# returaj/gan_mpc

Measured on AMD Instinct MI355X. Metric: trajectories/sec (rollout+backward+critic step) at batch=1024, H=50, higher is better.
Workload: dtype f32

## Files before the change

### gan_mpc_amd/csrc/gmpc_linearize_sparse.hip

```cpp
#include <cstdio>
#include <type_traits>

#include "gmpc_launch.h"

typedef float f32x4 __attribute__((ext_vector_type(4)));
typedef unsigned v4u __attribute__((ext_vector_type(4)));
typedef unsigned v2u __attribute__((ext_vector_type(2)));

#define GMPC_LIN_PADROWS 24
#define GMPC_SP_H 200
#define GMPC_SP_Z 200
#define GMPC_SP_STR 220
#define GMPC_SP_CAP 216
#define GMPC_SP_WAVE_BYTES (16 * GMPC_SP_STR * 4 + 3 * GMPC_SP_CAP * 4)
#define GMPC_SP_RD 3
#define GMPC_SP_ROW 256

static bool sparse_form(int L, const int* dims, int n, int m) {
  const int Lh = L - 1;
  if (Lh < 2 || n + m > 32 || n < 1) return false;
  for (int l = 1; l <= Lh; ++l)
    if (dims[l] != GMPC_SP_H) return false;
  return true;
}

__global__ void k_pack_sparse(const float* W, float* dst) {
  const int e = blockIdx.x * blockDim.x + threadIdx.x;
  if (e >= GMPC_SP_H * GMPC_SP_H) return;
  const int i = e / GMPC_SP_H, o = e - i * GMPC_SP_H;
  const int t = i >> 4;
  const int slot = i < 192 ? 64 * (t >> 2) + 4 * (i & 15) + (t & 3) : i;
  dst[(size_t)o * GMPC_SP_ROW + slot] = W[e];
}

size_t gmpc_linsparse_floats(int L, const int* dims, int n, int m) {
  if (!sparse_form(L, dims, n, m)) return 0;
  return (size_t)(L - 2) * (GMPC_SP_H + GMPC_LIN_PADROWS) * GMPC_SP_ROW + GMPC_SP_ROW;
}

void gmpc_linsparse_prepare(const MlpDesc& dyn, int n, int m, float* p, LinPad* out, hipStream_t s) {
  for (int l = 0; l < GMPC_MAX_LAYERS; ++l) out->WSP[l] = nullptr;
  if (!sparse_form(dyn.L, dyn.dims, n, m)) return;
  p = reinterpret_cast<float*>((reinterpret_cast<uintptr_t>(p) + 1023) & ~(uintptr_t)1023);
  for (int l = 1; l < dyn.L - 1; ++l) {
    out->WSP[l] = p;
    hipLaunchKernelGGL(k_pack_sparse, dim3((GMPC_SP_H * GMPC_SP_H + 255) / 256), dim3(256), 0, s, dyn.W[l], p);
    p += (size_t)(GMPC_SP_H + GMPC_LIN_PADROWS) * GMPC_SP_ROW;
  }
}

__global__ __launch_bounds__(GMPC_THREADS, 2) void k_linearize_sparse(
    int NSamp, int T, int n, int m, int Lh, LinPad lp, const uint32_t* masks, const int* active, float* AB,
    int samp_mul, int samp_add) {
  extern __shared__ __attribute__((aligned(16))) char smem[];
  const int lane = threadIdx.x & 63, wave = __builtin_amdgcn_readfirstlane(threadIdx.x >> 6);
  const int g = lane >> 4, l16 = lane & 15;
  const int nm = n + m;
  const int nrow = n < 16 ? n : 16;
  char* wbase = smem + wave * GMPC_SP_WAVE_BYTES;
  float* st = reinterpret_cast<float*>(wbase);
  unsigned* lk = reinterpret_cast<unsigned*>(wbase + 16 * GMPC_SP_STR * 4);
  unsigned* lt = lk + GMPC_SP_CAP;
  if (lane < 16 * 8) st[(lane >> 3) * GMPC_SP_STR + GMPC_SP_H + (lane & 7)] = 0.f;
  if (lane + 64 < 16 * 8) st[((lane + 64) >> 3) * GMPC_SP_STR + GMPC_SP_H + (lane & 7)] = 0.f;

  const int lw = l16 * 16, lwt = (192 + (l16 & 7)) * 4;
  const int ls = l16 * GMPC_SP_STR * 4;
  const int tsel = l16 >= 8 ? 1 : 0;
  const unsigned* lkl = lk + g;
  const unsigned* ltl_ = lt + 2 * g + tsel;
  const int lsn = l16 < n ? l16 * 4 : (1 << 28);
  const __amdgpu_buffer_rsrc_t rsl = __builtin_amdgcn_make_buffer_rsrc(
      const_cast<float*>(lp.WLP), 0, (GMPC_SP_H + GMPC_LIN_PADROWS) * n * (int)sizeof(float), 0x00020000);
  const __amdgpu_buffer_rsrc_t rs0 = __builtin_amdgcn_make_buffer_rsrc(
      const_cast<float*>(lp.WTP[0]), 0, (GMPC_SP_H + GMPC_LIN_PADROWS) * 32 * (int)sizeof(float), 0x00020000);

  constexpr int WPB = GMPC_THREADS / 64;
  for (int s = blockIdx.x * WPB + wave; s < NSamp; s += gridDim.x * WPB) {
    const size_t sid = (size_t)s * samp_mul + samp_add;
    if (active != nullptr && active[sid / T] == 0) continue;
    const uint32_t* mrow = masks + sid * Lh * GMPC_MW;

    auto build = [&](int ml) -> int {
      __builtin_amdgcn_wave_barrier();
      int base = 0;
#pragma unroll
      for (int c = 0; c < 4; ++c) {
        const uint32_t lo = __builtin_amdgcn_readfirstlane(mrow[ml * GMPC_MW + 2 * c]);
        uint32_t hi = c < 3 ? __builtin_amdgcn_readfirstlane(mrow[ml * GMPC_MW + 2 * c + 1]) : 0u;
        const uint32_t lo_m = c < 3 ? lo : (lo & 0xFFu);
        const uint32_t word = lane < 32 ? lo_m : hi;
        const int pos = base + (int)__builtin_amdgcn_mbcnt_hi(hi, __builtin_amdgcn_mbcnt_lo(lo_m, 0u));
        const unsigned u = 64 * c + lane;
        if ((word >> (lane & 31)) & 1u) {
          const bool odd = (u & 1u) != 0;
          lk[pos] = u;
          *reinterpret_cast<v2u*>(lt + 2 * pos) = v2u{odd ? GMPC_SP_Z : u, odd ? u : GMPC_SP_Z};
        }
        base += __builtin_popcount(lo_m) + __builtin_popcount(hi);
      }
      if (lane < 16) {
        lk[base + lane] = GMPC_SP_Z;
        *reinterpret_cast<v2u*>(lt + 2 * (base + lane)) = v2u{GMPC_SP_Z, GMPC_SP_Z};
      }
      __builtin_amdgcn_wave_barrier();
      return base;
    };

    auto layer = [&](int l, auto seedc) __attribute__((always_inline)) {
      constexpr bool seed = decltype(seedc)::value;
      const int np = (build(l) + 3) >> 2;
      const __amdgpu_buffer_rsrc_t wrs = __builtin_amdgcn_make_buffer_rsrc(
          const_cast<float*>(lp.WSP[l]), 0, (GMPC_SP_H + GMPC_LIN_PADROWS) * GMPC_SP_ROW * 4, 0x00020000);
      f32x4 acc[13];
      struct Ops { float w[13]; float b; unsigned k, kt; };
      Ops r[GMPC_SP_RD];
      auto tables = [&](Ops& o, int p) {
        o.k = lkl[4 * p];
        o.kt = ltl_[8 * p];
      };
      auto loads = [&](Ops& o) {
        const int k = (int)o.k, kt = (int)o.kt;
        const int vo = (k << 10) + lw, vt = (kt << 10) + lwt;
#pragma unroll
        for (int q = 0; q < 3; ++q) {
          const v4u a = __builtin_amdgcn_raw_buffer_load_b128(wrs, vo + 256 * q, 0, 0);
          o.w[4 * q] = __uint_as_float(a.x); o.w[4 * q + 1] = __uint_as_float(a.y);
          o.w[4 * q + 2] = __uint_as_float(a.z); o.w[4 * q + 3] = __uint_as_float(a.w);
        }
        o.w[12] = __uint_as_float(__builtin_amdgcn_raw_buffer_load_b32(wrs, vt, 0, 0));
        if constexpr (seed) o.b = __uint_as_float(__builtin_amdgcn_raw_buffer_load_b32(rsl, k * n * 4 + lsn, 0, 0));
        else o.b = st[(ls >> 2) + k];
      };
      auto step = [&](int p, Ops& cur, Ops& ahead2) __attribute__((always_inline)) {
        loads(ahead2);
        tables(cur, p + 3);
        __builtin_amdgcn_sched_barrier(0);
#pragma unroll
        for (int t = 0; t < 13; ++t) acc[t] = __builtin_amdgcn_mfma_f32_16x16x4f32(cur.w[t], cur.b, acc[t], 0, 0, 0);
        __builtin_amdgcn_sched_barrier(0);
      };
      if (np == 0) {
#pragma unroll
        for (int t = 0; t < 13; ++t) acc[t] = f32x4{0.f, 0.f, 0.f, 0.f};
      } else {
        tables(r[0], 0); tables(r[1], 1); tables(r[2], 2);
        loads(r[0]); loads(r[1]);
        loads(r[2]);
        tables(r[0], 3);
        __builtin_amdgcn_sched_barrier(0);
#pragma unroll
        for (int t = 0; t < 13; ++t)
          acc[t] = __builtin_amdgcn_mfma_f32_16x16x4f32(r[0].w[t], r[0].b, f32x4{0.f, 0.f, 0.f, 0.f}, 0, 0, 0);
        __builtin_amdgcn_sched_barrier(0);
        int p = 1;
        for (; p + 3 <= np; p += 3) {
          step(p, r[1], r[0]);
          step(p + 1, r[2], r[1]);
          step(p + 2, r[0], r[2]);
        }
        if (p < np) step(p, r[1], r[0]);
        if (p + 1 < np) step(p + 1, r[2], r[1]);
      }
      mfma_fence<false>(acc[0], acc[1], acc[2], acc[3], acc[4], acc[5], acc[6], acc[7], acc[8], acc[9], acc[10],
                        acc[11], acc[12]);
      __builtin_amdgcn_wave_barrier();
      float* srow = st + l16 * GMPC_SP_STR;
#pragma unroll
      for (int t = 0; t < 12; ++t)
        *reinterpret_cast<f32x4*>(srow + 32 * (t >> 1) + 16 * (t & 1) + 4 * g) = acc[t];
      *reinterpret_cast<f32x4*>(srow + (g < 2 ? 192 : 200) + 4 * g) = acc[12];
      __builtin_amdgcn_wave_barrier();
      if (g < 2) {
        const f32x4 x = *reinterpret_cast<const f32x4*>(srow + 192 + 4 * g);
        const f32x4 y = *reinterpret_cast<const f32x4*>(srow + 208 + 4 * g);
        *reinterpret_cast<f32x4*>(srow + 192 + 4 * g) = x + y;
      }
      __builtin_amdgcn_wave_barrier();
    };
    layer(Lh - 1, std::true_type{});
    for (int l = Lh - 2; l >= 1; --l) layer(l, std::false_type{});

    {
      const int np = (build(0) + 3) >> 2;
      f32x4 acc0 = {0.f, 0.f, 0.f, 0.f}, acc1 = {0.f, 0.f, 0.f, 0.f};
      const bool two = nm > 16;
      struct Ops0 { float w0, w1, b; unsigned k; };
      Ops0 r[GMPC_SP_RD];
      auto tables = [&](Ops0& o, int p) { o.k = lkl[4 * p]; };
      auto loads = [&](Ops0& o) {
        const int vo = (int)(o.k << 7) + l16 * 4;
        o.w0 = __uint_as_float(__builtin_amdgcn_raw_buffer_load_b32(rs0, vo, 0, 0));
        o.w1 = __uint_as_float(__builtin_amdgcn_raw_buffer_load_b32(rs0, vo + 64, 0, 0));
        o.b = st[(ls >> 2) + o.k];
      };
      auto step = [&](int p, Ops0& cur, Ops0& ahead2) __attribute__((always_inline)) {
        loads(ahead2);
        tables(cur, p + 3);
        __builtin_amdgcn_sched_barrier(0);
        acc0 = __builtin_amdgcn_mfma_f32_16x16x4f32(cur.w0, cur.b, acc0, 0, 0, 0);
        acc1 = __builtin_amdgcn_mfma_f32_16x16x4f32(cur.w1, cur.b, acc1, 0, 0, 0);
        __builtin_amdgcn_sched_barrier(0);
      };
      tables(r[0], 0); tables(r[1], 1); tables(r[2], 2);
      loads(r[0]); loads(r[1]);
      int p = 0;
      for (; p + 3 <= np; p += 3) {
        step(p, r[0], r[2]);
        step(p + 1, r[1], r[0]);
        step(p + 2, r[2], r[1]);
      }
      if (p < np) step(p, r[0], r[2]);
      if (p + 1 < np) step(p + 1, r[1], r[0]);
      mfma_fence<false>(acc0, acc1);
      if (l16 < nrow) {
        float* dst = AB + ((size_t)s * n + l16) * nm;
#pragma unroll
        for (int j = 0; j < 4; ++j) {
          const int c = 4 * g + j;
          if (c < nm) dst[c] = acc0[j] + (c == l16 ? 1.0f : 0.0f);
          if (two && c + 16 < nm) dst[c + 16] = acc1[j] + (c + 16 == l16 ? 1.0f : 0.0f);
        }
      }
    }
    __builtin_amdgcn_wave_barrier();
  }
}

int gmpc_launch_linearize_sparse(int NSamp, int T, int n, int m, const MlpDesc& dyn, const LinPad& lp,
                                 const uint32_t* masks, const int* active, float* AB, int samp_mul, int samp_add,
                                 hipStream_t s) {
  const int Lh = dyn.L - 1;
  if (!sparse_form(dyn.L, dyn.dims, n, m) || lp.NT != 7 || lp.NTF != 1 || lp.NGF != 1) return -1;
  if (NSamp <= 0) return 0;
  if (n > 16 && gmpc_launch_linearize_regs_rows(NSamp, T, n, m, dyn, lp, masks, active, AB, samp_mul, samp_add, 16,
                                                s) != 0)
    return -1;
  const size_t lds = (size_t)(GMPC_THREADS / 64) * GMPC_SP_WAVE_BYTES;
  int grid = (NSamp + 3) / 4;
  if (grid > 256 * 2) grid = 256 * 2;
  hipLaunchKernelGGL(k_linearize_sparse, dim3(grid), dim3(GMPC_THREADS), lds, s, NSamp, T, n, m, Lh, lp, masks,
                     active, AB, samp_mul, samp_add);
  return 0;
}
```

Measured before the change: 799,800.

## Software-pipeline sparse linearize across layers and samples with double-buffered index tables

Restructures the sparse linearization kernel so the next layer's (or next sample's) mask index table is built into a second LDS buffer and its first weight loads are issued while the current layer's last MFMAs run. Mask words are now loaded once per lane with a vector load and broadcast via readlane instead of scalar readfirstlane loads, and the next trajectory's active flag is prefetched. This targets the pipeline drain and refill bubble at every layer boundary and sample boundary. It doubles the per-wave index-table LDS footprint and adds considerable control complexity.

```diff
diff --git a/gan_mpc_amd/csrc/gmpc_linearize_sparse.hip b/gan_mpc_amd/csrc/gmpc_linearize_sparse.hip
--- a/gan_mpc_amd/csrc/gmpc_linearize_sparse.hip
+++ b/gan_mpc_amd/csrc/gmpc_linearize_sparse.hip
@@ -12,7 +12,7 @@
 #define GMPC_SP_Z 200
 #define GMPC_SP_STR 220
 #define GMPC_SP_CAP 216
-#define GMPC_SP_WAVE_BYTES (16 * GMPC_SP_STR * 4 + 3 * GMPC_SP_CAP * 4)
+#define GMPC_SP_WAVE_BYTES (16 * GMPC_SP_STR * 4 + 2 * 3 * GMPC_SP_CAP * 4)
 #define GMPC_SP_RD 3
 #define GMPC_SP_ROW 256
 
@@ -48,6 +48,10 @@
     p += (size_t)(GMPC_SP_H + GMPC_LIN_PADROWS) * GMPC_SP_ROW;
   }
 }
+
+struct SpOps { float w[13]; float b; unsigned k, kt; };
+enum { GMPC_SP_SEED = 0, GMPC_SP_HID = 1, GMPC_SP_INP = 2 };
+template <int V> using SpKind = std::integral_constant<int, V>;
 
 __global__ __launch_bounds__(GMPC_THREADS, 2) void k_linearize_sparse(
     int NSamp, int T, int n, int m, int Lh, LinPad lp, const uint32_t* masks, const int* active, float* AB,
@@ -59,109 +63,181 @@
   const int nrow = n < 16 ? n : 16;
   char* wbase = smem + wave * GMPC_SP_WAVE_BYTES;
   float* st = reinterpret_cast<float*>(wbase);
-  unsigned* lk = reinterpret_cast<unsigned*>(wbase + 16 * GMPC_SP_STR * 4);
-  unsigned* lt = lk + GMPC_SP_CAP;
+  unsigned* bc = reinterpret_cast<unsigned*>(wbase + 16 * GMPC_SP_STR * 4);
+  unsigned* bn = bc + 3 * GMPC_SP_CAP;
   if (lane < 16 * 8) st[(lane >> 3) * GMPC_SP_STR + GMPC_SP_H + (lane & 7)] = 0.f;
   if (lane + 64 < 16 * 8) st[((lane + 64) >> 3) * GMPC_SP_STR + GMPC_SP_H + (lane & 7)] = 0.f;
+  __builtin_amdgcn_wave_barrier();
 
   const int lw = l16 * 16, lwt = (192 + (l16 & 7)) * 4;
   const int ls = l16 * GMPC_SP_STR * 4;
   const int tsel = l16 >= 8 ? 1 : 0;
-  const unsigned* lkl = lk + g;
-  const unsigned* ltl_ = lt + 2 * g + tsel;
+  const int tofs = GMPC_SP_CAP + g + tsel;
   const int lsn = l16 < n ? l16 * 4 : (1 << 28);
   const __amdgpu_buffer_rsrc_t rsl = __builtin_amdgcn_make_buffer_rsrc(
       const_cast<float*>(lp.WLP), 0, (GMPC_SP_H + GMPC_LIN_PADROWS) * n * (int)sizeof(float), 0x00020000);
   const __amdgpu_buffer_rsrc_t rs0 = __builtin_amdgcn_make_buffer_rsrc(
       const_cast<float*>(lp.WTP[0]), 0, (GMPC_SP_H + GMPC_LIN_PADROWS) * 32 * (int)sizeof(float), 0x00020000);
-
-  constexpr int WPB = GMPC_THREADS / 64;
-  for (int s = blockIdx.x * WPB + wave; s < NSamp; s += gridDim.x * WPB) {
-    const size_t sid = (size_t)s * samp_mul + samp_add;
-    if (active != nullptr && active[sid / T] == 0) continue;
-    const uint32_t* mrow = masks + sid * Lh * GMPC_MW;
-
-    auto build = [&](int ml) -> int {
-      __builtin_amdgcn_wave_barrier();
-      int base = 0;
-#pragma unroll
-      for (int c = 0; c < 4; ++c) {
-        const uint32_t lo = __builtin_amdgcn_readfirstlane(mrow[ml * GMPC_MW + 2 * c]);
-        uint32_t hi = c < 3 ? __builtin_amdgcn_readfirstlane(mrow[ml * GMPC_MW + 2 * c + 1]) : 0u;
-        const uint32_t lo_m = c < 3 ? lo : (lo & 0xFFu);
-        const uint32_t word = lane < 32 ? lo_m : hi;
-        const int pos = base + (int)__builtin_amdgcn_mbcnt_hi(hi, __builtin_amdgcn_mbcnt_lo(lo_m, 0u));
-        const unsigned u = 64 * c + lane;
-        if ((word >> (lane & 31)) & 1u) {
-          const bool odd = (u & 1u) != 0;
-          lk[pos] = u;
-          *reinterpret_cast<v2u*>(lt + 2 * pos) = v2u{odd ? GMPC_SP_Z : u, odd ? u : GMPC_SP_Z};
+  auto wres = [&](int l) {
+    return __builtin_amdgcn_make_buffer_rsrc(const_cast<float*>(lp.WSP[l]), 0,
+                                             (GMPC_SP_H + GMPC_LIN_PADROWS) * GMPC_SP_ROW * 4, 0x00020000);
+  };
+
+  SpOps r[GMPC_SP_RD];
+  f32x4 acc[13];
+  constexpr SpKind<GMPC_SP_SEED> SEED{};
+  constexpr SpKind<GMPC_SP_HID> HID{};
+  constexpr SpKind<GMPC_SP_INP> INP{};
+
+  auto sample_id = [&](int sq) { return (size_t)sq * samp_mul + samp_add; };
+  auto traj_active = [&](int sq) { return active[sample_id(sq) / T] != 0; };
+  auto mask_words = [&](int sq, int ml) -> uint32_t {
+    return masks[(sample_id(sq) * Lh + ml) * GMPC_MW + (lane & 7)];
+  };
+
+  auto build = [&](uint32_t mwv, unsigned* b) -> int {
+    unsigned* lk = b;
+    unsigned* lt = b + GMPC_SP_CAP;
+    __builtin_amdgcn_wave_barrier();
+    int base = 0;
+#pragma unroll
+    for (int c = 0; c < 4; ++c) {
+      const uint32_t lo = (uint32_t)__builtin_amdgcn_readlane((int)mwv, 2 * c);
+      const uint32_t hi = c < 3 ? (uint32_t)__builtin_amdgcn_readlane((int)mwv, 2 * c + 1) : 0u;
+      const uint32_t lo_m = c < 3 ? lo : (lo & 0xFFu);
+      const uint32_t word = lane < 32 ? lo_m : hi;
+      const int pos = base + (int)__builtin_amdgcn_mbcnt_hi(hi, __builtin_amdgcn_mbcnt_lo(lo_m, 0u));
+      const unsigned u = 64 * c + lane;
+      if ((word >> (lane & 31)) & 1u) {
+        const bool odd = (u & 1u) != 0;
+        lk[pos] = u;
+        *reinterpret_cast<v2u*>(lt + 2 * pos) = v2u{odd ? GMPC_SP_Z : u, odd ? u : GMPC_SP_Z};
+      }
+      base += __builtin_popcount(lo_m) + __builtin_popcount(hi);
+    }
+    if (lane < 16) {
+      lk[base + lane] = GMPC_SP_Z;
+      *reinterpret_cast<v2u*>(lt + 2 * (base + lane)) = v2u{GMPC_SP_Z, GMPC_SP_Z};
+    }
+    __builtin_amdgcn_wave_barrier();
+    return base;
+  };
+
+  auto tables = [&](SpOps& o, const unsigned* b, int p, auto kind) {
+    const unsigned* ll = b + g;
+    o.k = ll[4 * p];
+    if constexpr (decltype(kind)::value != GMPC_SP_INP) o.kt = ll[tofs + 8 * p];
+  };
+  auto loads_a = [&](SpOps& o, const __amdgpu_buffer_rsrc_t rs, auto kind) {
+    constexpr int K = decltype(kind)::value;
+    const int k = (int)o.k;
+    if constexpr (K == GMPC_SP_INP) {
+      const int vo = (k << 7) + l16 * 4;
+      o.w[0] = __uint_as_float(__builtin_amdgcn_raw_buffer_load_b32(rs, vo, 0, 0));
+      o.w[1] = __uint_as_float(__builtin_amdgcn_raw_buffer_load_b32(rs, vo + 64, 0, 0));
+    } else {
+      const int kt = (int)o.kt;
+      const int vo = (k << 10) + lw, vt = (kt << 10) + lwt;
+#pragma unroll
+      for (int q = 0; q < 3; ++q) {
+        const v4u a = __builtin_amdgcn_raw_buffer_load_b128(rs, vo + 256 * q, 0, 0);
+        o.w[4 * q] = __uint_as_float(a.x); o.w[4 * q + 1] = __uint_as_float(a.y);
+        o.w[4 * q + 2] = __uint_as_float(a.z); o.w[4 * q + 3] = __uint_as_float(a.w);
+      }
+      o.w[12] = __uint_as_float(__builtin_amdgcn_raw_buffer_load_b32(rs, vt, 0, 0));
+      if constexpr (K == GMPC_SP_SEED)
+        o.b = __uint_as_float(__builtin_amdgcn_raw_buffer_load_b32(rsl, k * n * 4 + lsn, 0, 0));
+    }
+  };
+  auto loads_b = [&](SpOps& o, auto kind) {
+    if constexpr (decltype(kind)::value != GMPC_SP_SEED) o.b = st[(ls >> 2) + (int)o.k];
+  };
+  auto mfmas = [&](const SpOps& c, auto kind, auto first) __attribute__((always_inline)) {
+    constexpr int NT = decltype(kind)::value == GMPC_SP_INP ? 2 : 13;
+    __builtin_amdgcn_sched_barrier(0);
+#pragma unroll
+    for (int t = 0; t < NT; ++t)
+      acc[t] = __builtin_amdgcn_mfma_f32_16x16x4f32(
+          c.w[t], c.b, decltype(first)::value ? f32x4{0.f, 0.f, 0.f, 0.f} : acc[t], 0, 0, 0);
+    __builtin_amdgcn_sched_barrier(0);
+  };
+
+  auto phase = [&](auto kind, auto nkind, int np, const __amdgpu_buffer_rsrc_t rs, const __amdgpu_buffer_rsrc_t rsn,
+                   uint32_t mwv, int s) __attribute__((always_inline)) -> int {
+    constexpr int K = decltype(kind)::value;
+    constexpr std::false_type NO{};
+    constexpr std::true_type YES{};
+    int nl;
+    if (np >= 4) {
+      loads_b(r[0], kind); loads_b(r[1], kind); loads_b(r[2], kind);
+      auto step = [&](int p, SpOps& cur, SpOps& ahead2) __attribute__((always_inline)) {
+        loads_a(ahead2, rs, kind); loads_b(ahead2, kind);
+        tables(cur, bc, p + 3, kind);
+        mfmas(cur, kind, NO);
+      };
+      auto step0 = [&](SpOps& cur) __attribute__((always_inline)) {
+        tables(cur, bc, 3, kind);
+        mfmas(cur, kind, YES);
+      };
+      int p;
+      const int rem = np % 3;
+      if (rem == 1) {
+        step0(r[2]);
+        p = 1;
+      } else if (rem == 2) {
+        step0(r[1]);
+        step(1, r[2], r[1]);
+        p = 2;
+      } else {
+        step0(r[0]);
+        step(1, r[1], r[0]);
+        step(2, r[2], r[1]);
+        p = 3;
+      }
+      for (; p + 3 < np; p += 3) {
+        step(p, r[0], r[2]);
+        step(p + 1, r[1], r[0]);
+        step(p + 2, r[2], r[1]);
+      }
+      nl = build(mwv, bn);
+      const int j0 = ((nl + 3) >> 2) % 3, j1 = j0 == 2 ? 0 : j0 + 1, j2 = j1 == 2 ? 0 : j1 + 1;
+      loads_a(r[2], rs, kind); loads_b(r[2], kind);
+      tables(r[0], bn, j0, nkind);
+      mfmas(r[0], kind, NO);
+      loads_a(r[0], rsn, nkind);
+      tables(r[1], bn, j1, nkind);
+      mfmas(r[1], kind, NO);
+      loads_a(r[1], rsn, nkind);
+      tables(r[2], bn, j2, nkind);
+      mfmas(r[2], kind, NO);
+      loads_a(r[2], rsn, nkind);
+    } else {
+      constexpr int NT = K == GMPC_SP_INP ? 2 : 13;
+#pragma unroll
+      for (int t = 0; t < NT; ++t) acc[t] = f32x4{0.f, 0.f, 0.f, 0.f};
+      for (int p = 0; p < np; ++p) {
+        tables(r[0], bc, p, kind);
+        loads_a(r[0], rs, kind); loads_b(r[0], kind);
+        mfmas(r[0], kind, NO);
+      }
+      nl = build(mwv, bn);
+      const int j0 = ((nl + 3) >> 2) % 3, j1 = j0 == 2 ? 0 : j0 + 1, j2 = j1 == 2 ? 0 : j1 + 1;
+      tables(r[0], bn, j0, nkind); tables(r[1], bn, j1, nkind); tables(r[2], bn, j2, nkind);
+      loads_a(r[0], rsn, nkind); loads_a(r[1], rsn, nkind); loads_a(r[2], rsn, nkind);
+    }
+    if constexpr (K == GMPC_SP_INP) {
+      mfma_fence<false>(acc[0], acc[1]);
+      const bool two = nm > 16;
+      if (l16 < nrow) {
+        float* dst = AB + ((size_t)s * n + l16) * nm;
+#pragma unroll
+        for (int j = 0; j < 4; ++j) {
+          const int c = 4 * g + j;
+          if (c < nm) dst[c] = acc[0][j] + (c == l16 ? 1.0f : 0.0f);
+          if (two && c + 16 < nm) dst[c + 16] = acc[1][j] + (c + 16 == l16 ? 1.0f : 0.0f);
         }
-        base += __builtin_popcount(lo_m) + __builtin_popcount(hi);
-      }
-      if (lane < 16) {
-        lk[base + lane] = GMPC_SP_Z;
-        *reinterpret_cast<v2u*>(lt + 2 * (base + lane)) = v2u{GMPC_SP_Z, GMPC_SP_Z};
-      }
-      __builtin_amdgcn_wave_barrier();
-      return base;
-    };
-
-    auto layer = [&](int l, auto seedc) __attribute__((always_inline)) {
-      constexpr bool seed = decltype(seedc)::value;
-      const int np = (build(l) + 3) >> 2;
-      const __amdgpu_buffer_rsrc_t wrs = __builtin_amdgcn_make_buffer_rsrc(
-          const_cast<float*>(lp.WSP[l]), 0, (GMPC_SP_H + GMPC_LIN_PADROWS) * GMPC_SP_ROW * 4, 0x00020000);
-      f32x4 acc[13];
-      struct Ops { float w[13]; float b; unsigned k, kt; };
-      Ops r[GMPC_SP_RD];
-      auto tables = [&](Ops& o, int p) {
-        o.k = lkl[4 * p];
-        o.kt = ltl_[8 * p];
-      };
-      auto loads = [&](Ops& o) {
-        const int k = (int)o.k, kt = (int)o.kt;
-        const int vo = (k << 10) + lw, vt = (kt << 10) + lwt;
-#pragma unroll
-        for (int q = 0; q < 3; ++q) {
-          const v4u a = __builtin_amdgcn_raw_buffer_load_b128(wrs, vo + 256 * q, 0, 0);
-          o.w[4 * q] = __uint_as_float(a.x); o.w[4 * q + 1] = __uint_as_float(a.y);
-          o.w[4 * q + 2] = __uint_as_float(a.z); o.w[4 * q + 3] = __uint_as_float(a.w);
-        }
-        o.w[12] = __uint_as_float(__builtin_amdgcn_raw_buffer_load_b32(wrs, vt, 0, 0));
-        if constexpr (seed) o.b = __uint_as_float(__builtin_amdgcn_raw_buffer_load_b32(rsl, k * n * 4 + lsn, 0, 0));
-        else o.b = st[(ls >> 2) + k];
-      };
-      auto step = [&](int p, Ops& cur, Ops& ahead2) __attribute__((always_inline)) {
-        loads(ahead2);
-        tables(cur, p + 3);
-        __builtin_amdgcn_sched_barrier(0);
-#pragma unroll
-        for (int t = 0; t < 13; ++t) acc[t] = __builtin_amdgcn_mfma_f32_16x16x4f32(cur.w[t], cur.b, acc[t], 0, 0, 0);
-        __builtin_amdgcn_sched_barrier(0);
-      };
-      if (np == 0) {
-#pragma unroll
-        for (int t = 0; t < 13; ++t) acc[t] = f32x4{0.f, 0.f, 0.f, 0.f};
-      } else {
-        tables(r[0], 0); tables(r[1], 1); tables(r[2], 2);
-        loads(r[0]); loads(r[1]);
-        loads(r[2]);
-        tables(r[0], 3);
-        __builtin_amdgcn_sched_barrier(0);
-#pragma unroll
-        for (int t = 0; t < 13; ++t)
-          acc[t] = __builtin_amdgcn_mfma_f32_16x16x4f32(r[0].w[t], r[0].b, f32x4{0.f, 0.f, 0.f, 0.f}, 0, 0, 0);
-        __builtin_amdgcn_sched_barrier(0);
-        int p = 1;
-        for (; p + 3 <= np; p += 3) {
-          step(p, r[1], r[0]);
-          step(p + 1, r[2], r[1]);
-          step(p + 2, r[0], r[2]);
-        }
-        if (p < np) step(p, r[1], r[0]);
-        if (p + 1 < np) step(p + 1, r[2], r[1]);
-      }
+      }
+    } else {
       mfma_fence<false>(acc[0], acc[1], acc[2], acc[3], acc[4], acc[5], acc[6], acc[7], acc[8], acc[9], acc[10],
                         acc[11], acc[12]);
       __builtin_amdgcn_wave_barrier();
@@ -176,54 +252,51 @@
         const f32x4 y = *reinterpret_cast<const f32x4*>(srow + 208 + 4 * g);
         *reinterpret_cast<f32x4*>(srow + 192 + 4 * g) = x + y;
       }
-      __builtin_amdgcn_wave_barrier();
-    };
-    layer(Lh - 1, std::true_type{});
-    for (int l = Lh - 2; l >= 1; --l) layer(l, std::false_type{});
-
-    {
-      const int np = (build(0) + 3) >> 2;
-      f32x4 acc0 = {0.f, 0.f, 0.f, 0.f}, acc1 = {0.f, 0.f, 0.f, 0.f};
-      const bool two = nm > 16;
-      struct Ops0 { float w0, w1, b; unsigned k; };
-      Ops0 r[GMPC_SP_RD];
-      auto tables = [&](Ops0& o, int p) { o.k = lkl[4 * p]; };
-      auto loads = [&](Ops0& o) {
-        const int vo = (int)(o.k << 7) + l16 * 4;
-        o.w0 = __uint_as_float(__builtin_amdgcn_raw_buffer_load_b32(rs0, vo, 0, 0));
-        o.w1 = __uint_as_float(__builtin_amdgcn_raw_buffer_load_b32(rs0, vo + 64, 0, 0));
-        o.b = st[(ls >> 2) + o.k];
-      };
-      auto step = [&](int p, Ops0& cur, Ops0& ahead2) __attribute__((always_inline)) {
-        loads(ahead2);
-        tables(cur, p + 3);
-        __builtin_amdgcn_sched_barrier(0);
-        acc0 = __builtin_amdgcn_mfma_f32_16x16x4f32(cur.w0, cur.b, acc0, 0, 0, 0);
-        acc1 = __builtin_amdgcn_mfma_f32_16x16x4f32(cur.w1, cur.b, acc1, 0, 0, 0);
-        __builtin_amdgcn_sched_barrier(0);
-      };
-      tables(r[0], 0); tables(r[1], 1); tables(r[2], 2);
-      loads(r[0]); loads(r[1]);
-      int p = 0;
-      for (; p + 3 <= np; p += 3) {
-        step(p, r[0], r[2]);
-        step(p + 1, r[1], r[0]);
-        step(p + 2, r[2], r[1]);
-      }
-      if (p < np) step(p, r[0], r[2]);
-      if (p + 1 < np) step(p + 1, r[1], r[0]);
-      mfma_fence<false>(acc0, acc1);
-      if (l16 < nrow) {
-        float* dst = AB + ((size_t)s * n + l16) * nm;
-#pragma unroll
-        for (int j = 0; j < 4; ++j) {
-          const int c = 4 * g + j;
-          if (c < nm) dst[c] = acc0[j] + (c == l16 ? 1.0f : 0.0f);
-          if (two && c + 16 < nm) dst[c + 16] = acc1[j] + (c + 16 == l16 ? 1.0f : 0.0f);
-        }
-      }
     }
     __builtin_amdgcn_wave_barrier();
+    unsigned* t = bc; bc = bn; bn = t;
+    return (nl + 3) >> 2;
+  };
+
+  constexpr int WPB = GMPC_THREADS / 64;
+  const int stride = gridDim.x * WPB;
+  int s = blockIdx.x * WPB + wave;
+  if (active != nullptr)
+    while (s < NSamp && !traj_active(s)) s += stride;
+  if (s >= NSamp) return;
+  int np;
+  {
+    const int nl = build(mask_words(s, Lh - 1), bn);
+    const int j0 = ((nl + 3) >> 2) % 3, j1 = j0 == 2 ? 0 : j0 + 1, j2 = j1 == 2 ? 0 : j1 + 1;
+    const __amdgpu_buffer_rsrc_t rsn = wres(Lh - 1);
+    tables(r[0], bn, j0, SEED); tables(r[1], bn, j1, SEED); tables(r[2], bn, j2, SEED);
+    loads_a(r[0], rsn, SEED); loads_a(r[1], rsn, SEED); loads_a(r[2], rsn, SEED);
+    unsigned* t = bc; bc = bn; bn = t;
+    np = (nl + 3) >> 2;
+  }
+  for (;;) {
+    int sn = s + stride;
+    int av = 1;
+    if (active != nullptr && sn < NSamp) {
+      int vz = 0;
+      asm volatile("" : "+v"(vz));
+      av = active[sample_id(sn) / T + vz];
+    }
+    if (Lh > 2) np = phase(SEED, HID, np, wres(Lh - 1), wres(Lh - 2), mask_words(s, Lh - 2), s);
+    else np = phase(SEED, INP, np, wres(Lh - 1), rs0, mask_words(s, 0), s);
+    for (int l = Lh - 2; l >= 1; --l) {
+      if (l > 1) np = phase(HID, HID, np, wres(l), wres(l - 1), mask_words(s, l - 1), s);
+      else np = phase(HID, INP, np, wres(l), rs0, mask_words(s, 0), s);
+    }
+    if (active != nullptr && sn < NSamp && __builtin_amdgcn_readfirstlane(av) == 0) {
+      do sn += stride;
+      while (sn < NSamp && !traj_active(sn));
+    }
+    uint32_t mwv = 0u;
+    if (sn < NSamp) mwv = mask_words(sn, Lh - 1);
+    np = phase(INP, SEED, np, rs0, wres(Lh - 1), mwv, s);
+    if (sn >= NSamp) break;
+    s = sn;
   }
 }
 
```

After: 798,900. Within noise of the previous version (-0.1%).
